# yihua7/NeRF-Texture

Measured on AMD Instinct MI355X. Metric: ray-samples/s (train), higher is better.
Workload: dtype f16

## Files before the change

nerf-texture_amd/csrc/common.hpp:

```cpp
#pragma once

#include <hip/hip_runtime.h>
#include <hip/hip_fp16.h>
#include <stdint.h>

#include <cstdarg>
#include <cstdio>

#include "../../include/nerftex_hip.h"

namespace nerftex {

void set_error(const char* fmt, ...);
void clear_error();

inline hipStream_t as_stream(void* s) { return reinterpret_cast<hipStream_t>(s); }

inline int check_launch(const char* what) {
    hipError_t e = hipGetLastError();
    if (e != hipSuccess) {
        set_error("%s: HIP launch failed: %s", what, hipGetErrorString(e));
        return NERFTEX_ERR_HIP;
    }
    return NERFTEX_OK;
}

#define NERFTEX_HIP_TRY(expr, what)                                                   \
    do {                                                                              \
        hipError_t _e = (expr);                                                       \
        if (_e != hipSuccess) {                                                       \
            ::nerftex::set_error("%s: %s", what, hipGetErrorString(_e));              \
            return NERFTEX_ERR_HIP;                                                   \
        }                                                                             \
    } while (0)

template <typename T>
constexpr T div_up(T a, T b) { return (a + b - 1) / b; }

inline int device_cus() {
    static int cus[16] = {0};
    int dev = 0;
    if (hipGetDevice(&dev) != hipSuccess || dev < 0 || dev >= 16) return 256;
    if (cus[dev] == 0) {
        hipDeviceProp_t prop;
        cus[dev] = (hipGetDeviceProperties(&prop, dev) == hipSuccess && prop.multiProcessorCount > 0) ? prop.multiProcessorCount : 256;
    }
    return cus[dev];
}

enum Knob {
    kKnobGridFwd,
    kKnobGridBwd,
    kKnobGridBwdSweep,
    kKnobGridBwdItems,
    kKnobGridBwdSlice,
    kKnobGridBwdNoMerge,
    kKnobGridBwdProbe,
    kKnobMarch,
    kKnobMarchSerial,
    kKnobFfmlpWgPerCu,
    kKnobFfmlpBwdSplit,
    kKnobMarchLean,
    kKnobFfmlpBwdTr,
    kKnobGridBwdStage,
    kKnobCompositeKeep,
    kKnobMarchCountProbe,
    kKnobPlanarLanes,
    kKnobPatchLanes,
    kKnobCount
};
extern long g_knobs[kKnobCount];
inline long knob(Knob k) { return g_knobs[k]; }

extern int g_profile_mode;
constexpr int kTimeAny = 1, kTimeGrid = 2;
void profile_begin(const char* name, hipStream_t st, int* slot);
void profile_end(hipStream_t st, int slot);
struct KernelTimer {
    hipStream_t st;
    int slot = -1;
    KernelTimer(const char* name, hipStream_t s, int group = kTimeAny) : st(s) {
        if (g_profile_mode == 1 || (g_profile_mode == 2 && group == kTimeGrid)) profile_begin(name, s, &slot);
    }
    ~KernelTimer() { if (slot >= 0) profile_end(st, slot); }
};

using half_t = _Float16;
typedef _Float16 half2_t __attribute__((ext_vector_type(2)));
typedef _Float16 half4_t __attribute__((ext_vector_type(4)));
typedef _Float16 half8_t __attribute__((ext_vector_type(8)));
typedef float float2_t __attribute__((ext_vector_type(2)));
typedef float float4_t __attribute__((ext_vector_type(4)));
typedef float float16_t __attribute__((ext_vector_type(16)));

constexpr int kWave = 64;

__host__ __device__ __forceinline__ uint32_t unit_rows(uint32_t code, uint32_t count) {
    if (!(code >> 31)) return code;
    const uint32_t F = (code >> 24) & 127u, N = code & 0xffffffu;
    const uint32_t q = F * N / (count ? count : 1u);
    return q < F ? F : (q > 8u * F ? 8u * F : q);
}
__device__ __forceinline__ uint32_t live_rows(uint32_t B, const int32_t* __restrict__ units_dev, uint32_t rows_per_unit) {
    if (!units_dev) return B;
    const uint32_t n = (uint32_t)units_dev[0];
    return min(B, n * unit_rows(rows_per_unit, n));
}
__device__ __forceinline__ bool slot_unused(const float* __restrict__ dirs, size_t row) { return dirs[row * 3] > 1e29f; }

}
```

nerf-texture_amd/csrc/ffmlp_body.inc:

```

constexpr int kBlockThreads = 256;
constexpr int kTilesPerWave = 2;
constexpr int kRowsPerBlock = 4 * 16 * kTilesPerWave;
constexpr float kAct = 10.0f;

enum Act : uint32_t { kRelu = 0, kExp = 1, kSine = 2, kSigmoid = 3, kSquareplus = 4, kSoftplus = 5, kNone = 6 };

__device__ __forceinline__ float act_forward(uint32_t a, float x) {
    switch (a) {
        case kRelu: return __builtin_bit_cast(float, max(__builtin_bit_cast(int, x), 0));
        case kExp: return expf(x);
        case kSine: return sinf(x);
        case kSigmoid: return 1.0f / (1.0f + expf(-x));
        case kSquareplus: { const float s = x * kAct; return 0.5f * (s + sqrtf(s * s + 4.0f)) / kAct; }
        case kSoftplus: return logf(expf(x * kAct) + 1.0f) / kAct;
        default: return x;
    }
}
__device__ __forceinline__ float act_backward(uint32_t a, float g, float y) {
    switch (a) {
        case kRelu: return y > 0.0f ? g : 0.0f;
        case kExp: return g * y;
        case kSigmoid: return g * (float)(elem_t)(y * (1.0f - y));
        case kSquareplus: { const float s = y * kAct; return g * (float)(elem_t)(s * s / (s * s + 1.0f)); }
        case kSoftplus: return g * (float)(elem_t)(1.0f - expf(-y * kAct));
        default: return g;
    }
}

template <int ACT>
__device__ __forceinline__ float act_fwd(uint32_t act_rt, float x) {
    if constexpr (ACT >= 0) return act_forward((uint32_t)ACT, x);
    else return act_forward(act_rt, x);
}
template <int ACT>
__device__ __forceinline__ float act_bwd(uint32_t act_rt, float g, float y) {
    if constexpr (ACT >= 0) return act_backward((uint32_t)ACT, g, y);
    else return act_backward(act_rt, g, y);
}


__device__ __forceinline__ int kmap(bool permuted, int ks, int g, int j) {
    return permuted ? 32 * ks + 16 * (j >> 2) + 4 * g + (j & 3) : 32 * ks + 8 * g + j;
}

__device__ void stage_fragments(elem8_t* __restrict__ dst, const elem_t* __restrict__ W, int ldw, bool transposed, int M, int K,
                                bool permuted) {
    const int KS = (K + 31) / 32;
    const elem8_t zero8{0, 0, 0, 0, 0, 0, 0, 0};
    if (!transposed) {
        const int total = (M / 16) * KS * 64;
        for (int s = threadIdx.x; s < total; s += kBlockThreads) {
            const int frag = s >> 6, lane = s & 63;
            const int mt = frag / KS, ks = frag - mt * KS;
            const int m = 16 * mt + (lane & 15), g = lane >> 4;
            const elem_t* row = W + (size_t)m * ldw;
            elem8_t v;
            if (!permuted) {
                const int k0 = 32 * ks + 8 * g;
                v = k0 < K ? *reinterpret_cast<const elem8_t*>(row + k0) : zero8;
            } else {
                const int ka = 32 * ks + 4 * g, kb = ka + 16;
                const elem4_t z4{0, 0, 0, 0};
                const elem4_t lo = ka < K ? *reinterpret_cast<const elem4_t*>(row + ka) : z4;
                const elem4_t hi = kb < K ? *reinterpret_cast<const elem4_t*>(row + kb) : z4;
                v = elem8_t{lo[0], lo[1], lo[2], lo[3], hi[0], hi[1], hi[2], hi[3]};
            }
            dst[s] = v;
        }
    } else {
        elem_t* d = reinterpret_cast<elem_t*>(dst);
        const int MP = M / 8;
        for (int s = threadIdx.x; s < KS * 32 * MP; s += kBlockThreads) {
            const int k = s / MP, m0 = 8 * (s - k * MP);
            const elem8_t v = k < K ? *reinterpret_cast<const elem8_t*>(W + (size_t)k * ldw + m0) : zero8;
            const int ks = k >> 5, kk = k & 31;
            const int g = permuted ? (kk & 15) >> 2 : kk >> 3;
            const int j = permuted ? 4 * (kk >> 4) + (kk & 3) : kk & 7;
#pragma unroll
            for (int i = 0; i < 8; i++) {
                const int m = m0 + i;
                d[((size_t)((m >> 4) * KS + ks) * 64 + (m & 15) + 16 * g) * 8 + j] = v[i];
            }
        }
    }
}

__host__ __device__ constexpr int frag_count(int M, int K) { return (M / 16) * ((K + 31) / 32); }

__device__ __forceinline__ elem8_t pack_operand(const float4_t& lo, const float4_t& hi) {
    elem8_t b;
#pragma unroll
    for (int j = 0; j < 4; j++) {
        b[j] = (elem_t)lo[j];
        b[4 + j] = (elem_t)hi[j];
    }
    return b;
}

__device__ __forceinline__ void store4(elem_t* p, const float4_t& v) {
    elem4_t h;
#pragma unroll
    for (int j = 0; j < 4; j++) h[j] = (elem_t)v[j];
    *reinterpret_cast<elem4_t*>(p) = h;
}

template <int HIDDEN, bool INFERENCE, bool STAGED, int ACT, int OUT_ACT, bool STREAM = false, bool ROWS = false>
__global__ __launch_bounds__(kBlockThreads) void ffmlp_forward_kernel(const elem_t* __restrict__ X, const elem_t* __restrict__ W,
                                                                      elem_t* __restrict__ fwd, elem_t* __restrict__ out, uint32_t B,
                                                                      uint32_t IN, uint32_t NL, uint32_t act, uint32_t out_act,
                                                                      const int32_t* __restrict__ units_dev, uint32_t rows_per_unit) {
    constexpr int OT = HIDDEN / 16;
    constexpr int KSH = (HIDDEN + 31) / 32;
    constexpr int NT = kTilesPerWave;
    uint32_t live = B;
    if constexpr (ROWS) {
        live = live_rows(B, units_dev, rows_per_unit);
        if (blockIdx.x * kRowsPerBlock >= live) return;
    }
    extern __shared__ __attribute__((aligned(16))) char smem[];
    elem8_t* frags = reinterpret_cast<elem8_t*>(smem);

    const int KS0 = (IN + 31) / 32;
    const int base_hidden = OT * KS0;
    const int per_hidden = OT * KSH;
    const int base_out = base_hidden + (NL - 1) * per_hidden;
    const size_t patch_offset = (size_t)(base_out + KSH) * 1024;
    static_assert(!(STREAM && STAGED), "the streaming form stores its activations directly (the LDS holds one layer's fragments and nothing else)");
    if constexpr (!STREAM) {
        stage_fragments(frags, W, IN, false, HIDDEN, IN, false);
        for (uint32_t l = 1; l < NL; l++)
            stage_fragments(frags + (size_t)(base_hidden + (l - 1) * per_hidden) * 64, W + (size_t)HIDDEN * IN + (size_t)(l - 1) * HIDDEN * HIDDEN,
                            HIDDEN, false, HIDDEN, HIDDEN, true);
        stage_fragments(frags + (size_t)base_out * 64, W + (size_t)HIDDEN * IN + (size_t)(NL - 1) * HIDDEN * HIDDEN, HIDDEN, false, 16, HIDDEN,
                        true);
        __syncthreads();
    }
    auto fragments_of = [&](uint32_t m) -> const elem8_t* {
        if constexpr (STREAM) {
            __syncthreads();
            if (m == 0) stage_fragments(frags, W, IN, false, HIDDEN, IN, false);
            else if (m < NL) stage_fragments(frags, W + (size_t)HIDDEN * IN + (size_t)(m - 1) * HIDDEN * HIDDEN, HIDDEN, false, HIDDEN, HIDDEN, true);
            else stage_fragments(frags, W + (size_t)HIDDEN * IN + (size_t)(NL - 1) * HIDDEN * HIDDEN, HIDDEN, false, 16, HIDDEN, true);
            __syncthreads();
            return frags;
        } else {
            return m == 0 ? frags : (m < NL ? frags + (size_t)(base_hidden + (m - 1) * per_hidden) * 64 : frags + (size_t)base_out * 64);
        }
    };

    const int wave = threadIdx.x >> 6, lane = threadIdx.x & 63, r = lane & 15, g = lane >> 4;
    const size_t layer_stride = (size_t)B * HIDDEN;
    constexpr int kRowPitch = HIDDEN + 8;
    elem_t* patch = reinterpret_cast<elem_t*>(smem + patch_offset) + (size_t)wave * 16 * NT * kRowPitch;

    for (uint32_t row0 = blockIdx.x * kRowsPerBlock + wave * 16 * NT; ROWS ? row0 - wave * 16 * NT < live : row0 < B; row0 += gridDim.x * kRowsPerBlock) {
        float4_t acc[NT][OT];
#pragma unroll
        for (int t = 0; t < NT; t++)
#pragma unroll
            for (int ot = 0; ot < OT; ot++) acc[t][ot] = float4_t{0, 0, 0, 0};

        const elem8_t* f0 = fragments_of(0);
        for (int ks = 0; ks < KS0; ks++) {
            elem8_t b[NT];
            const uint32_t k0 = 32 * ks + 8 * g;
#pragma unroll
            for (int t = 0; t < NT; t++) {
                if (k0 < IN) b[t] = *reinterpret_cast<const elem8_t*>(X + (size_t)(row0 + 16 * t + r) * IN + k0);
                else b[t] = elem8_t{0, 0, 0, 0, 0, 0, 0, 0};
            }
#pragma unroll
            for (int ot = 0; ot < OT; ot++) {
                const elem8_t a = f0[(size_t)(ot * KS0 + ks) * 64 + lane];
#pragma unroll
                for (int t = 0; t < NT; t++) acc[t][ot] = mfma16(a, b[t], acc[t][ot]);
            }
        }

        elem8_t bop[NT][KSH];
        for (uint32_t l = 0;; l++) {
#pragma unroll
            for (int t = 0; t < NT; t++) {
#pragma unroll
                for (int ot = 0; ot < OT; ot++) {
#pragma unroll
                    for (int j = 0; j < 4; j++) acc[t][ot][j] = act_fwd<ACT>(act, acc[t][ot][j]);
                    if constexpr (!INFERENCE) {
                        if constexpr (STAGED) store4(patch + (size_t)(16 * t + r) * kRowPitch + 16 * ot + 4 * g, acc[t][ot]);
                        else store4(fwd + l * layer_stride + (size_t)(row0 + 16 * t + r) * HIDDEN + 16 * ot + 4 * g, acc[t][ot]);
                    }
                }
#pragma unroll
                for (int s = 0; s < KSH; s++) {
                    const float4_t zero{0, 0, 0, 0};
                    bop[t][s] = pack_operand(acc[t][2 * s], (2 * s + 1 < OT) ? acc[t][(2 * s + 1 < OT) ? 2 * s + 1 : 0] : zero);
                }
            }
            if constexpr (!INFERENCE && STAGED) {
                constexpr int kPieces = HIDDEN / 8;
                elem_t* dst = fwd + l * layer_stride + (size_t)row0 * HIDDEN;
#pragma unroll
                for (int it = 0; it < 16 * NT * kPieces / 64; it++) {
                    const int c = it * 64 + lane, row = c / kPieces, piece = c % kPieces;
                    *reinterpret_cast<elem8_t*>(dst + (size_t)row * HIDDEN + 8 * piece) =
                        *reinterpret_cast<const elem8_t*>(patch + (size_t)row * kRowPitch + 8 * piece);
                }
            }
            if (l + 1 >= NL) break;
            const elem8_t* fl = fragments_of(l + 1);
#pragma unroll
            for (int ot = 0; ot < OT; ot++) {
                float4_t c[NT];
#pragma unroll
                for (int t = 0; t < NT; t++) c[t] = float4_t{0, 0, 0, 0};
#pragma unroll
                for (int ks = 0; ks < KSH; ks++) {
                    const elem8_t a = fl[(size_t)(ot * KSH + ks) * 64 + lane];
#pragma unroll
                    for (int t = 0; t < NT; t++) c[t] = mfma16(a, bop[t][ks], c[t]);
                }
#pragma unroll
                for (int t = 0; t < NT; t++) acc[t][ot] = c[t];
            }
        }

        {
            const elem8_t* fo = fragments_of(NL);
            float4_t c[NT];
#pragma unroll
            for (int t = 0; t < NT; t++) c[t] = float4_t{0, 0, 0, 0};
#pragma unroll
            for (int ks = 0; ks < KSH; ks++) {
                const elem8_t a = fo[(size_t)ks * 64 + lane];
#pragma unroll
                for (int t = 0; t < NT; t++) c[t] = mfma16(a, bop[t][ks], c[t]);
            }
#pragma unroll
            for (int t = 0; t < NT; t++) {
#pragma unroll
                for (int j = 0; j < 4; j++) c[t][j] = act_fwd<OUT_ACT>(out_act, c[t][j]);
                store4(out + (size_t)(row0 + 16 * t + r) * 16 + 4 * g, c[t]);
            }
        }
    }
}

__device__ __forceinline__ elem_t narrow16(float v) {
    asm volatile("" : "+v"(v));
    return (elem_t)v;
}

template <bool TRAIN, bool DENSITY = false>
__global__ __launch_bounds__(kBlockThreads) void field_forward_kernel(const elem_t* __restrict__ feats, const float* __restrict__ dirs,
                                                                      const elem_t* __restrict__ Ws, const elem_t* __restrict__ Wc, uint32_t B,
                                                                      float* __restrict__ sigma, float* __restrict__ rgbs, elem_t* __restrict__ x_rows,
                                                                      elem_t* __restrict__ h_out, elem_t* __restrict__ cin_out,
                                                                      elem_t* __restrict__ hc_out, const int* __restrict__ units_dev,
                                                                      uint32_t rows_per_unit) {
    constexpr int HIDDEN = 64, IN = 32, OT = 4, KSH = 2, NT = kTilesPerWave;
    const uint32_t live = units_dev ? min(B, (uint32_t)units_dev[0] * unit_rows(rows_per_unit, (uint32_t)units_dev[0])) : B;
    extern __shared__ __attribute__((aligned(16))) char smem[];
    elem8_t* frags = reinterpret_cast<elem8_t*>(smem);
    constexpr int kS0 = 0, kS1 = 4, kSo = 12, kC0 = 14, kC1 = 18, kC2 = 26, kCo = 34;
    stage_fragments(frags + kS0 * 64, Ws, IN, false, HIDDEN, IN, false);
    stage_fragments(frags + kS1 * 64, Ws + HIDDEN * IN, HIDDEN, false, HIDDEN, HIDDEN, true);
    stage_fragments(frags + kSo * 64, Ws + HIDDEN * IN + HIDDEN * HIDDEN, HIDDEN, false, 16, HIDDEN, true);
    if constexpr (!DENSITY) {
        stage_fragments(frags + kC0 * 64, Wc, IN, false, HIDDEN, IN, false);
        stage_fragments(frags + kC1 * 64, Wc + HIDDEN * IN, HIDDEN, false, HIDDEN, HIDDEN, true);
        stage_fragments(frags + kC2 * 64, Wc + HIDDEN * IN + HIDDEN * HIDDEN, HIDDEN, false, HIDDEN, HIDDEN, true);
        stage_fragments(frags + kCo * 64, Wc + HIDDEN * IN + 2 * HIDDEN * HIDDEN, HIDDEN, false, 16, HIDDEN, true);
    }
    __syncthreads();

    const int wave = threadIdx.x >> 6, lane = threadIdx.x & 63, r = lane & 15, g = lane >> 4;
    auto hidden = [&](const elem8_t* fl, const elem8_t (&bop)[NT][KSH], float4_t (&acc)[NT][OT]) {
#pragma unroll
        for (int ot = 0; ot < OT; ot++) {
            float4_t c[NT];
#pragma unroll
            for (int t = 0; t < NT; t++) c[t] = float4_t{0, 0, 0, 0};
#pragma unroll
            for (int ks = 0; ks < KSH; ks++) {
                const elem8_t a = fl[(size_t)(ot * KSH + ks) * 64 + lane];
#pragma unroll
                for (int t = 0; t < NT; t++) c[t] = mfma16(a, bop[t][ks], c[t]);
            }
#pragma unroll
            for (int t = 0; t < NT; t++) acc[t][ot] = c[t];
        }
    };
    auto relu_pack = [&](float4_t (&acc)[NT][OT], elem8_t (&bop)[NT][KSH]) {
#pragma unroll
        for (int t = 0; t < NT; t++) {
#pragma unroll
            for (int ot = 0; ot < OT; ot++)
#pragma unroll
                for (int j = 0; j < 4; j++) acc[t][ot][j] = act_forward(kRelu, acc[t][ot][j]);
#pragma unroll
            for (int s = 0; s < KSH; s++) bop[t][s] = pack_operand(acc[t][2 * s], acc[t][2 * s + 1]);
        }
    };
    auto out_tile = [&](const elem8_t* fo, const elem8_t (&bop)[NT][KSH], float4_t (&c)[NT]) {
#pragma unroll
        for (int t = 0; t < NT; t++) c[t] = float4_t{0, 0, 0, 0};
#pragma unroll
        for (int ks = 0; ks < KSH; ks++) {
            const elem8_t a = fo[(size_t)ks * 64 + lane];
#pragma unroll
            for (int t = 0; t < NT; t++) c[t] = mfma16(a, bop[t][ks], c[t]);
        }
    };

    for (uint32_t row0 = blockIdx.x * kRowsPerBlock + wave * 16 * NT; row0 < live; row0 += gridDim.x * kRowsPerBlock) {
        if constexpr (!TRAIN && !DENSITY) {
            bool used = false;
#pragma unroll
            for (int t = 0; t < NT; t++) used |= !(dirs[(size_t)(row0 + 16 * t + r) * 3] > 1e29f);
            if (__ballot(used) == 0ull) continue;
        }
        float4_t acc[NT][OT];
        elem8_t bop[NT][KSH];
        {
            elem8_t b[NT];
#pragma unroll
            for (int t = 0; t < NT; t++) {
                const size_t row = row0 + 16 * t + r;
                uint32_t w[4];
#pragma unroll
                for (int q = 0; q < 4; q++) w[q] = *reinterpret_cast<const uint32_t*>(feats + ((size_t)(4 * g + q) * B + row) * 2);
                typedef uint32_t u4 __attribute__((ext_vector_type(4)));
                if constexpr (kElemIsHalf) {
                    b[t] = __builtin_bit_cast(elem8_t, u4{w[0], w[1], w[2], w[3]});
                } else {
                    const half8_t hf = __builtin_bit_cast(half8_t, u4{w[0], w[1], w[2], w[3]});
#pragma unroll
                    for (int j = 0; j < 8; j++) b[t][j] = (elem_t)(float)hf[j];
                }
                if constexpr (TRAIN) *reinterpret_cast<elem8_t*>(x_rows + row * IN + 8 * g) = b[t];
            }
#pragma unroll
            for (int ot = 0; ot < OT; ot++) {
                const elem8_t a = frags[(size_t)(kS0 + ot) * 64 + lane];
#pragma unroll
                for (int t = 0; t < NT; t++) acc[t][ot] = mfma16(a, b[t], float4_t{0, 0, 0, 0});
            }
        }
        relu_pack(acc, bop);
        hidden(frags + kS1 * 64, bop, acc);
        relu_pack(acc, bop);
        float4_t h[NT];
        out_tile(frags + kSo * 64, bop, h);

        if constexpr (DENSITY) {
            if (g == 0) {
#pragma unroll
                for (int t = 0; t < NT; t++) sigma[row0 + 16 * t + r] = expf((float)(elem_t)h[t][0]);
            }
            continue;
        }
        elem8_t bc[NT];
#pragma unroll
        for (int t = 0; t < NT; t++) {
            const size_t row = row0 + 16 * t + r;
            float4_t hr;
#pragma unroll
            for (int j = 0; j < 4; j++) hr[j] = (float)(elem_t)h[t][j];
            if (g == 0) sigma[row] = expf(hr[0]);
            float sh16[16];
            sh::eval<4>(dirs[row * 3], dirs[row * 3 + 1], dirs[row * 3 + 2], sh16);
            elem8_t cv;
#pragma unroll
            for (int j = 0; j < 8; j++) {
                const float geo = __shfl(hr[(j + 1) & 3], r + 16 * (2 * (g & 1) + ((j + 1) >> 2)), 64);
                float sh_lo = sh16[j], sh_hi = sh16[8 + j];
                asm volatile("" : "+v"(sh_lo), "+v"(sh_hi));
                const float shj = (g & 1) ? sh_hi : sh_lo;
                cv[j] = g < 2 ? narrow16(shj) : ((g == 3 && j == 7) ? (elem_t)0.0f : (elem_t)geo);
            }
            bc[t] = cv;
            if constexpr (TRAIN) {
                store4(h_out + row * 16 + 4 * g, h[t]);
                *reinterpret_cast<elem8_t*>(cin_out + row * IN + 8 * g) = cv;
            }
        }
#pragma unroll
        for (int ot = 0; ot < OT; ot++) {
            const elem8_t a = frags[(size_t)(kC0 + ot) * 64 + lane];
#pragma unroll
            for (int t = 0; t < NT; t++) acc[t][ot] = mfma16(a, bc[t], float4_t{0, 0, 0, 0});
        }
        relu_pack(acc, bop);
        hidden(frags + kC1 * 64, bop, acc);
        relu_pack(acc, bop);
        hidden(frags + kC2 * 64, bop, acc);
        relu_pack(acc, bop);
        float4_t c[NT];
        out_tile(frags + kCo * 64, bop, c);
#pragma unroll
        for (int t = 0; t < NT; t++) {
            const size_t row = row0 + 16 * t + r;
            if constexpr (TRAIN)
                if (hc_out) store4(hc_out + row * 16 + 4 * g, c[t]);
            if (g == 0) {
#pragma unroll
                for (int k = 0; k < 3; k++) {
                    const float x = (float)(elem_t)c[t][k];
                    rgbs[row * 3 + k] = (float)narrow16(1.0f / (1.0f + expf(-x)));
                }
            }
        }
    }
}

template <int HIDDEN, bool STREAM = false>
__global__ __launch_bounds__(kBlockThreads) void ffmlp_dgrad_kernel(const elem_t* __restrict__ grad, const elem_t* __restrict__ W,
                                                                    const elem_t* __restrict__ fwd, elem_t* __restrict__ bb,
                                                                    elem_t* __restrict__ grad_inputs, uint32_t B, uint32_t IN, uint32_t NL,
                                                                    uint32_t act) {
    constexpr int OT = HIDDEN / 16;
    constexpr int KSH = (HIDDEN + 31) / 32;
    constexpr int NT = kTilesPerWave;
    extern __shared__ __attribute__((aligned(16))) char smem[];
    elem8_t* frags = reinterpret_cast<elem8_t*>(smem);

    const elem_t* W_hidden = W + (size_t)HIDDEN * IN;
    const elem_t* W_out = W_hidden + (size_t)(NL - 1) * HIDDEN * HIDDEN;
    const int per_hidden = OT * KSH;
    const int base_hidden = OT;
    const int base_in = base_hidden + (NL - 1) * per_hidden;
    if constexpr (!STREAM) {
        stage_fragments(frags, W_out, HIDDEN, true, HIDDEN, 16, false);
        for (uint32_t j = 1; j < NL; j++)
            stage_fragments(frags + (size_t)(base_hidden + (j - 1) * per_hidden) * 64, W_hidden + (size_t)(NL - 1 - j) * HIDDEN * HIDDEN, HIDDEN, true,
                            HIDDEN, HIDDEN, true);
        if (grad_inputs) stage_fragments(frags + (size_t)base_in * 64, W, IN, true, IN, HIDDEN, true);
        __syncthreads();
    }
    auto fragments_of = [&](uint32_t j) -> const elem8_t* {
        if constexpr (STREAM) {
            __syncthreads();
            if (j == 0) stage_fragments(frags, W_out, HIDDEN, true, HIDDEN, 16, false);
            else if (j < NL) stage_fragments(frags, W_hidden + (size_t)(NL - 1 - j) * HIDDEN * HIDDEN, HIDDEN, true, HIDDEN, HIDDEN, true);
            else stage_fragments(frags, W, IN, true, IN, HIDDEN, true);
            __syncthreads();
            return frags;
        } else {
            return j == 0 ? frags : (j < NL ? frags + (size_t)(base_hidden + (j - 1) * per_hidden) * 64 : frags + (size_t)base_in * 64);
        }
    };

    const int wave = threadIdx.x >> 6, lane = threadIdx.x & 63, r = lane & 15, g = lane >> 4;
    const size_t layer_stride = (size_t)B * HIDDEN;

    for (uint32_t row0 = blockIdx.x * kRowsPerBlock + wave * 16 * NT; row0 < B; row0 += gridDim.x * kRowsPerBlock) {
        elem8_t bg[NT];
#pragma unroll
        for (int t = 0; t < NT; t++) {
            if (g < 2) bg[t] = *reinterpret_cast<const elem8_t*>(grad + (size_t)(row0 + 16 * t + r) * 16 + 8 * g);
            else bg[t] = elem8_t{0, 0, 0, 0, 0, 0, 0, 0};
        }
        float4_t acc[NT][OT];
        const elem8_t* fout = fragments_of(0);
#pragma unroll
        for (int ot = 0; ot < OT; ot++) {
            const elem8_t a = fout[(size_t)ot * 64 + lane];
#pragma unroll
            for (int t = 0; t < NT; t++) acc[t][ot] = mfma16(a, bg[t], float4_t{0, 0, 0, 0});
        }

        elem8_t bop[NT][KSH];
        for (uint32_t j = 0;; j++) {
            const elem_t* f = fwd + (size_t)(NL - 1 - j) * layer_stride;
#pragma unroll
            for (int t = 0; t < NT; t++) {
#pragma unroll
                for (int ot = 0; ot < OT; ot++) {
                    const size_t off = (size_t)(row0 + 16 * t + r) * HIDDEN + 16 * ot + 4 * g;
                    const elem4_t y = *reinterpret_cast<const elem4_t*>(f + off);
#pragma unroll
                    for (int q = 0; q < 4; q++) acc[t][ot][q] = act_backward(act, (float)(elem_t)acc[t][ot][q], (float)y[q]);
                    store4(bb + j * layer_stride + off, acc[t][ot]);
                }
#pragma unroll
                for (int s = 0; s < KSH; s++) {
                    const float4_t zero{0, 0, 0, 0};
                    bop[t][s] = pack_operand(acc[t][2 * s], (2 * s + 1 < OT) ? acc[t][(2 * s + 1 < OT) ? 2 * s + 1 : 0] : zero);
                }
            }
            if (j + 1 >= NL) break;
            const elem8_t* fl = fragments_of(j + 1);
#pragma unroll
            for (int ot = 0; ot < OT; ot++) {
                float4_t c[NT];
// ... 918 lines not shown
        return NERFTEX_ERR_INVALID;
    }
    return dispatch_forward<false>(inputs, weights, B, input_dim, hidden_dim, num_layers, activation, output_activation, forward_buffer, outputs,
                                   as_stream(stream));
}

int inference_entry(const void* inputs, const void* weights, uint32_t B, uint32_t input_dim, uint32_t output_dim,
                                       uint32_t hidden_dim, uint32_t num_layers, uint32_t activation, uint32_t output_activation,
                                       void* inference_buffer, void* outputs, void* stream) {
    (void)inference_buffer;
    clear_error();
    int rc = validate(B, input_dim, output_dim, hidden_dim, num_layers, activation, output_activation);
    if (rc != NERFTEX_OK || B == 0) return rc;
    if ((rc = weights_aligned(weights)) != NERFTEX_OK) return rc;
    return dispatch_forward<true>(inputs, weights, B, input_dim, hidden_dim, num_layers, activation, output_activation, nullptr, outputs,
                                  as_stream(stream));
}

int backward_entry(const void* grad, const void* inputs, const void* weights, const void* forward_buffer, uint32_t B,
                                      uint32_t input_dim, uint32_t output_dim, uint32_t hidden_dim, uint32_t num_layers, uint32_t activation,
                                      uint32_t output_activation, int calc_grad_inputs, void* backward_buffer, void* grad_inputs,
                                      void* grad_weights, void* stream) {
    clear_error();
    int rc = validate(B, input_dim, output_dim, hidden_dim, num_layers, activation, output_activation);
    if (rc != NERFTEX_OK || B == 0) return rc;
    if ((rc = weights_aligned(weights)) != NERFTEX_OK) return rc;

    hipStream_t st = as_stream(stream);
    const uint32_t H = hidden_dim, IN = input_dim, NL = num_layers;
    void* gi = calc_grad_inputs ? grad_inputs : nullptr;
    const uint32_t n_params = H * (IN + H * (NL - 1) + 16);

    {
        if (!knob(kKnobFfmlpBwdSplit)) {
            rc = launch_backward_fused(grad, inputs, weights, forward_buffer, gi, B, IN, H, NL, activation, n_params, grad_weights, st);
            if (rc >= 0) return rc;
        }
    }
    if (!backward_buffer || !forward_buffer) {
        set_error("ffmlp_backward: forward_buffer and backward_buffer must not be NULL for this shape / mode");
        return NERFTEX_ERR_INVALID;
    }

    switch (H) {
        case 16: rc = launch_dgrad<16>(grad, weights, forward_buffer, backward_buffer, gi, B, IN, NL, activation, st); break;
        case 32: rc = launch_dgrad<32>(grad, weights, forward_buffer, backward_buffer, gi, B, IN, NL, activation, st); break;
        case 64: rc = launch_dgrad<64>(grad, weights, forward_buffer, backward_buffer, gi, B, IN, NL, activation, st); break;
        case 128: rc = launch_dgrad<128>(grad, weights, forward_buffer, backward_buffer, gi, B, IN, NL, activation, st); break;
        default: rc = launch_dgrad<256>(grad, weights, forward_buffer, backward_buffer, gi, B, IN, NL, activation, st); break;
    }
    if (rc != NERFTEX_OK) return rc;

    const size_t LS = (size_t)B * H;
    const elem_t* fb = static_cast<const elem_t*>(forward_buffer);
    const elem_t* bb = static_cast<const elem_t*>(backward_buffer);
    WgradArgs args{};
    args.layer[0] = WgradLayer{bb + (size_t)(NL - 1) * LS, static_cast<const elem_t*>(inputs), H, IN, H, IN, 0};
    for (uint32_t l = 1; l < NL; l++)
        args.layer[l] = WgradLayer{bb + (size_t)(NL - 1 - l) * LS, fb + (size_t)(l - 1) * LS, H, H, H, H, H * IN + (l - 1) * H * H};
    args.layer[NL] = WgradLayer{static_cast<const elem_t*>(grad), fb + (size_t)(NL - 1) * LS, 16, H, 16, H, H * IN + (NL - 1) * H * H};

    uint32_t n_parts = B / 128;
    const uint32_t cap = (uint32_t)num_cus() / 2;
    if (n_parts > cap) n_parts = cap;
    if (n_parts == 0) n_parts = 1;
    float* partials = static_cast<float*>(workspace(kWsMlp, sizeof(float) * (size_t)n_parts * n_params, st));
    if (!partials) return NERFTEX_ERR_HIP;
    const size_t red_bytes = sizeof(float) * 4 * 16 * 256;
    {
        KernelTimer kt("ffmlp_wgrad_kernel", st);
        hipLaunchKernelGGL(ffmlp_wgrad_kernel, dim3(n_parts, NL + 1), dim3(kBlockThreads), red_bytes, st, args, B, partials, n_params);
    }
    rc = check_launch("ffmlp_backward(wgrad)");
    if (rc != NERFTEX_OK) return rc;
    {
        KernelTimer kt("ffmlp_wgrad_reduce_kernel", st);
        hipLaunchKernelGGL(ffmlp_wgrad_reduce_kernel, dim3(div_up(n_params, kRedParams)), dim3(kBlockThreads), 0, st, partials, n_parts,
                           n_params, static_cast<elem_t*>(grad_weights));
    }
    return check_launch("ffmlp_backward(reduce)");
}


int field_density_entry(const void* feats_lbc, const void* sigma_weights, uint32_t B, float* sigma, void* stream) {
    clear_error();
    if (B % kRowsPerBlock != 0) {
        set_error("field_density: the batch must be a multiple of %d rows", kRowsPerBlock);
        return NERFTEX_ERR_INVALID;
    }
    if (B == 0) return NERFTEX_OK;
    int rc = weights_aligned(sigma_weights);
    if (rc != NERFTEX_OK) return rc;
    const size_t lds = (size_t)14 * 1024;
    hipStream_t st = as_stream(stream);
    {
        KernelTimer kt("field_density_kernel", st);
        hipLaunchKernelGGL((field_forward_kernel<false, true>), dim3(persistent_grid(B, lds)), dim3(kBlockThreads), lds, st, (const elem_t*)feats_lbc,
                           (const float*)nullptr, (const elem_t*)sigma_weights, (const elem_t*)nullptr, B, sigma, (float*)nullptr, (elem_t*)nullptr,
                           (elem_t*)nullptr, (elem_t*)nullptr, (elem_t*)nullptr, (const int*)nullptr, 0u);
    }
    return check_launch("field_density");
}

int field_forward_entry(const void* feats_lbc, const float* dirs, const void* sigma_weights, const void* color_weights, uint32_t B, float* sigma,
                        float* rgbs, void* x_rows, void* h, void* cin, void* hc, const int32_t* units_dev, uint32_t rows_per_unit, void* stream) {
    clear_error();
    if (B % kRowsPerBlock != 0) {
        set_error("field_forward: the batch must be a multiple of %d rows", kRowsPerBlock);
        return NERFTEX_ERR_INVALID;
    }
    const bool train = x_rows || h || cin || hc;
    if (train && !(x_rows && h && cin)) {
        set_error("field_forward: x_rows, h and cin (and optionally hc) are written together (training) or not at all (inference)");
        return NERFTEX_ERR_INVALID;
    }
    if (B == 0) return NERFTEX_OK;
    int rc = weights_aligned(sigma_weights);
    if (rc == NERFTEX_OK) rc = weights_aligned(color_weights);
    if (rc != NERFTEX_OK) return rc;
    const size_t lds = (size_t)36 * 1024;
    auto kernel = train ? field_forward_kernel<true> : field_forward_kernel<false>;
    hipStream_t st = as_stream(stream);
    {
        KernelTimer kt(train ? "field_forward_train_kernel" : "field_forward_kernel", st);
        hipLaunchKernelGGL(kernel, dim3(persistent_grid(B, lds)), dim3(kBlockThreads), lds, st, (const elem_t*)feats_lbc, dirs, (const elem_t*)sigma_weights,
                           (const elem_t*)color_weights, B, sigma, rgbs, (elem_t*)x_rows, (elem_t*)h, (elem_t*)cin, (elem_t*)hc, units_dev, rows_per_unit);
    }
    return check_launch("field_forward");
}
```

nerf-texture_amd/csrc/runtime.hip:

```cpp
#include "common.hpp"
#include "workspace.hpp"

#include <atomic>

#include <cstdlib>
#include <cstring>
#include <map>
#include <mutex>
#include <string>
#include <vector>

namespace nerftex {

static thread_local char g_err[512] = {0};

void set_error(const char* fmt, ...) {
    va_list ap;
    va_start(ap, fmt);
    vsnprintf(g_err, sizeof(g_err), fmt, ap);
    va_end(ap);
}

void clear_error() { g_err[0] = 0; }

long g_knobs[kKnobCount] = {0};
namespace {
const char* const kKnobNames[kKnobCount] = {"grid_fwd", "grid_bwd", "grid_bwd_sweep", "grid_bwd_items", "grid_bwd_slice", "grid_bwd_nomerge",
                                            "grid_bwd_probe", "march", "march_serial", "ffmlp_wg_per_cu",
                                            "ffmlp_bwd_split", "march_lean", "ffmlp_bwd_tr", "grid_bwd_stage", "composite_keep", "march_count_probe", "planar_lanes",
                                            "patch_lanes"};
int knob_index(const char* name, size_t n) {
    for (int k = 0; k < kKnobCount; k++)
        if (strlen(kKnobNames[k]) == n && strncmp(kKnobNames[k], name, n) == 0) return k;
    return -1;
}
struct KnobInit {
    KnobInit() {
        auto env = [](const char* n) { const char* v = getenv(n); return v ? v : ""; };
        const char* v;
        v = env("NERFTEX_GRID_FWD"); g_knobs[kKnobGridFwd] = v[0] == 'p' ? 1 : v[0] == 'l' ? 2 : 0;
        v = env("NERFTEX_GRID_BWD"); g_knobs[kKnobGridBwd] = v[0] == 'a' ? 1 : v[0] == 'o' ? 2 : 0;
        g_knobs[kKnobGridBwdSweep] = env("NERFTEX_GRID_BWD_ALGO")[0] == 's';
        g_knobs[kKnobGridBwdItems] = atol(env("NERFTEX_GRID_BWD_ITEMS"));
        g_knobs[kKnobGridBwdSlice] = atol(env("NERFTEX_GRID_BWD_SLICE"));
        g_knobs[kKnobGridBwdNoMerge] = getenv("NERFTEX_GRID_BWD_NOMERGE") != nullptr;
        v = env("NERFTEX_MARCH"); g_knobs[kKnobMarch] = v[0] == 'r' ? 1 : v[0] == 'l' ? 2 : 0;
        g_knobs[kKnobMarchSerial] = env("NERFTEX_MARCH_COUNT")[0] == 's';
        g_knobs[kKnobFfmlpWgPerCu] = atol(env("NERFTEX_FFMLP_WG_PER_CU"));
        g_knobs[kKnobFfmlpBwdSplit] = env("NERFTEX_FFMLP_BWD")[0] == 's';
        for (const char* p = env("NERFTEX_TUNE"); *p;) {
            const char* eq = strchr(p, '=');
            if (!eq) break;
            const int k = knob_index(p, (size_t)(eq - p));
            if (k >= 0) g_knobs[k] = atol(eq + 1);
            const char* c = strchr(eq, ',');
            if (!c) break;
            p = c + 1;
        }
    }
} g_knob_init;
}

namespace {
constexpr int kMaxDevices = 16;
struct Slot { void* ptr = nullptr; size_t bytes = 0; };
struct SlotSet { Slot slot[kWsSlots]; };
std::map<hipStream_t, SlotSet> g_ws[kMaxDevices];
const hipStream_t kCaptureSet = reinterpret_cast<hipStream_t>(~(uintptr_t)0);
std::vector<void*> g_retired;
std::mutex g_ws_mutex;
}

std::atomic<unsigned> g_ws_touched{0};
thread_local int t_capture_set = 0;

void* workspace(WorkspaceSlot slot, size_t bytes, hipStream_t stream) {
    g_ws_touched.fetch_or(1u << (unsigned)slot, std::memory_order_relaxed);
    int dev = 0;
    if (hipGetDevice(&dev) != hipSuccess || dev < 0 || dev >= kMaxDevices) {
        set_error("workspace: bad device");
        return nullptr;
    }
    hipStreamCaptureStatus cap = hipStreamCaptureStatusNone;
    if (hipStreamIsCapturing(stream, &cap) == hipSuccess && cap != hipStreamCaptureStatusNone)
        stream = reinterpret_cast<hipStream_t>(reinterpret_cast<uintptr_t>(kCaptureSet) - (uintptr_t)t_capture_set);
    std::lock_guard<std::mutex> lock(g_ws_mutex);
    Slot& s = g_ws[dev][stream].slot[slot];
    if (s.bytes < bytes) {
        if (s.ptr) g_retired.push_back(s.ptr);
        s.ptr = nullptr;
        s.bytes = 0;
        size_t want = bytes < (1u << 20) ? (1u << 20) : bytes + bytes / 2;
        hipStreamCaptureMode mode = hipStreamCaptureModeRelaxed;
        (void)hipThreadExchangeStreamCaptureMode(&mode);
        const hipError_t err = hipMalloc(&s.ptr, want);
        (void)hipThreadExchangeStreamCaptureMode(&mode);
        if (err != hipSuccess) {
            set_error("workspace: hipMalloc(%zu) failed", want);
            s.ptr = nullptr;
            return nullptr;
        }
        s.bytes = want;
        static const int poison = [] { const char* v = getenv("NERFTEX_POISON_WORKSPACE"); return v && *v ? atoi(v) : -1; }();
        if (poison >= 0) {
            (void)hipThreadExchangeStreamCaptureMode(&mode);
            (void)hipMemset(s.ptr, poison & 255, want);
            (void)hipThreadExchangeStreamCaptureMode(&mode);
        }
    }
    return s.ptr;
}

bool peek_workspace(int slot, hipStream_t stream, void** ptr, size_t* bytes) {
// ... 147 lines not shown
```

Measured before the change: 938.6 million.

## Prefetch next rows and stage weight fragments directly in field forward kernel

Restructures the fused field MLP forward kernel so each wave loads its weight fragments straight from global memory into LDS slots instead of the generic staging loop. Features and directions for the next grid-stride step are prefetched while the current step computes. Blocks with no live rows exit early. Spherical-harmonic packing is done once per step via permlane32 swaps, and the geometry features are shuffled as packed halves, cutting per-tile shuffles and conversions. It also adds compile-time probe variants, selected by a knob that defaults to off. The risks are higher register pressure from the prefetch buffers and a changed LDS layout.

```diff
diff --git a/nerf-texture_amd/csrc/common.hpp b/nerf-texture_amd/csrc/common.hpp
--- a/nerf-texture_amd/csrc/common.hpp
+++ b/nerf-texture_amd/csrc/common.hpp
@@ -67,6 +67,7 @@
     kKnobMarchCountProbe,
     kKnobPlanarLanes,
     kKnobPatchLanes,
+    kKnobFieldFwdProbe,
     kKnobCount
 };
 extern long g_knobs[kKnobCount];
diff --git a/nerf-texture_amd/csrc/ffmlp_body.inc b/nerf-texture_amd/csrc/ffmlp_body.inc
--- a/nerf-texture_amd/csrc/ffmlp_body.inc
+++ b/nerf-texture_amd/csrc/ffmlp_body.inc
@@ -88,6 +88,19 @@
 
 __host__ __device__ constexpr int frag_count(int M, int K) { return (M / 16) * ((K + 31) / 32); }
 
+template <int KS, bool PERMUTED>
+__device__ __forceinline__ elem8_t fragment_slot(const elem_t* __restrict__ W, int ldw, int f, int lane) {
+    const int mt = f / KS, ks = f - mt * KS;
+    const elem_t* row = W + (size_t)(16 * mt + (lane & 15)) * ldw + 32 * ks;
+    const int g = lane >> 4;
+    if constexpr (!PERMUTED) {
+        return *reinterpret_cast<const elem8_t*>(row + 8 * g);
+    } else {
+        const elem4_t lo = *reinterpret_cast<const elem4_t*>(row + 4 * g), hi = *reinterpret_cast<const elem4_t*>(row + 4 * g + 16);
+        return elem8_t{lo[0], lo[1], lo[2], lo[3], hi[0], hi[1], hi[2], hi[3]};
+    }
+}
+
 __device__ __forceinline__ elem8_t pack_operand(const float4_t& lo, const float4_t& hi) {
     elem8_t b;
 #pragma unroll
@@ -251,7 +264,12 @@
     return (elem_t)v;
 }
 
-template <bool TRAIN, bool DENSITY = false>
+enum FieldProbe : int { kProbeOff = 0, kProbeStaging = 1, kProbeLoads = 2, kProbeSigma = 3, kProbeMid = 4, kProbeColour = 5, kProbeCount = 6 };
+typedef uint32_t uint4_t __attribute__((ext_vector_type(4)));
+__device__ __forceinline__ void probe_sink(const elem8_t& v) { asm volatile("" ::"v"(__builtin_bit_cast(uint4_t, v))); }
+__device__ __forceinline__ void probe_sink(const float4_t& v) { asm volatile("" ::"v"(v)); }
+
+template <bool TRAIN, bool DENSITY = false, int PROBE = kProbeOff>
 __global__ __launch_bounds__(kBlockThreads) void field_forward_kernel(const elem_t* __restrict__ feats, const float* __restrict__ dirs,
                                                                       const elem_t* __restrict__ Ws, const elem_t* __restrict__ Wc, uint32_t B,
                                                                       float* __restrict__ sigma, float* __restrict__ rgbs, elem_t* __restrict__ x_rows,
@@ -259,22 +277,76 @@
                                                                       elem_t* __restrict__ hc_out, const int* __restrict__ units_dev,
                                                                       uint32_t rows_per_unit) {
     constexpr int HIDDEN = 64, IN = 32, OT = 4, KSH = 2, NT = kTilesPerWave;
+    constexpr bool SKIP = !TRAIN && !DENSITY;
     const uint32_t live = units_dev ? min(B, (uint32_t)units_dev[0] * unit_rows(rows_per_unit, (uint32_t)units_dev[0])) : B;
+    if (blockIdx.x * kRowsPerBlock >= live) return;
     extern __shared__ __attribute__((aligned(16))) char smem[];
     elem8_t* frags = reinterpret_cast<elem8_t*>(smem);
-    constexpr int kS0 = 0, kS1 = 4, kSo = 12, kC0 = 14, kC1 = 18, kC2 = 26, kCo = 34;
-    stage_fragments(frags + kS0 * 64, Ws, IN, false, HIDDEN, IN, false);
-    stage_fragments(frags + kS1 * 64, Ws + HIDDEN * IN, HIDDEN, false, HIDDEN, HIDDEN, true);
-    stage_fragments(frags + kSo * 64, Ws + HIDDEN * IN + HIDDEN * HIDDEN, HIDDEN, false, 16, HIDDEN, true);
-    if constexpr (!DENSITY) {
-        stage_fragments(frags + kC0 * 64, Wc, IN, false, HIDDEN, IN, false);
-        stage_fragments(frags + kC1 * 64, Wc + HIDDEN * IN, HIDDEN, false, HIDDEN, HIDDEN, true);
-        stage_fragments(frags + kC2 * 64, Wc + HIDDEN * IN + HIDDEN * HIDDEN, HIDDEN, false, HIDDEN, HIDDEN, true);
-        stage_fragments(frags + kCo * 64, Wc + HIDDEN * IN + 2 * HIDDEN * HIDDEN, HIDDEN, false, 16, HIDDEN, true);
+
+    const int wave = __builtin_amdgcn_readfirstlane(threadIdx.x >> 6), lane = threadIdx.x & 63, r = lane & 15, g = lane >> 4;
+    const uint32_t stride = gridDim.x * kRowsPerBlock;
+    struct Feat { uint32_t w[NT][4]; };
+    struct Dir { float x, y, z; };
+    auto load_feats = [&](uint32_t row0) {
+        Feat f;
+#pragma unroll
+        for (int t = 0; t < NT; t++)
+#pragma unroll
+            for (int q = 0; q < 4; q++) f.w[t][q] = *reinterpret_cast<const uint32_t*>(feats + ((size_t)(4 * g + q) * B + row0 + 16 * t + r) * 2);
+        return f;
+    };
+    auto load_dir = [&](uint32_t row0) {
+        Dir d{0.0f, 0.0f, 0.0f};
+        if constexpr (!DENSITY) {
+            const size_t row = row0 + 16 * (g >> 1) + r;
+            d = Dir{dirs[row * 3], dirs[row * 3 + 1], dirs[row * 3 + 2]};
+        }
+        return d;
+    };
+    auto step_used = [&](const Dir& d) {
+        if constexpr (SKIP) return __ballot(!(d.x > 1e29f)) != 0ull;
+        else return true;
+    };
+    uint32_t row0 = blockIdx.x * kRowsPerBlock + wave * 16 * NT, row1 = row0 + stride;
+    const bool any_step = row0 < live;
+    if (!any_step) row0 = row1 = blockIdx.x * kRowsPerBlock;
+    Dir d_cur = load_dir(row0), d_nxt = load_dir(row1 < live ? row1 : row0);
+    bool used_cur = step_used(d_cur);
+    Feat w_cur = load_feats(row0);
+
+    constexpr int kS0 = 0, kS1 = 4, kC0 = 12, kC1 = 16, kC2 = 24, kSo = DENSITY ? 12 : 32, kCo = 34;
+    {
+        constexpr int kGroups = DENSITY ? 4 : 9;
+        const elem_t* const Ws1 = Ws + HIDDEN * IN;
+        const elem_t* const Wso = Ws1 + HIDDEN * HIDDEN;
+        elem8_t fv[kGroups];
+        fv[0] = fragment_slot<1, false>(Ws, IN, wave, lane);
+        fv[1] = fragment_slot<2, true>(Ws1, HIDDEN, wave, lane);
+        fv[2] = fragment_slot<2, true>(Ws1, HIDDEN, 4 + wave, lane);
+        if constexpr (DENSITY) {
+            fv[3] = fragment_slot<2, true>(Wso, HIDDEN, wave & 1, lane);
+        } else {
+            const elem_t* const Wc1 = Wc + HIDDEN * IN;
+            const elem_t* const Wc2 = Wc1 + HIDDEN * HIDDEN;
+            fv[3] = fragment_slot<1, false>(Wc, IN, wave, lane);
+            fv[4] = fragment_slot<2, true>(Wc1, HIDDEN, wave, lane);
+            fv[5] = fragment_slot<2, true>(Wc1, HIDDEN, 4 + wave, lane);
+            fv[6] = fragment_slot<2, true>(Wc2, HIDDEN, wave, lane);
+            fv[7] = fragment_slot<2, true>(Wc2, HIDDEN, 4 + wave, lane);
+            fv[8] = fragment_slot<2, true>(wave < 2 ? Wso : Wc2 + HIDDEN * HIDDEN, HIDDEN, wave & 1, lane);
+        }
+#pragma unroll
+        for (int t = 0; t < NT; t++)
+#pragma unroll
+            for (int q = 0; q < 4; q++) asm volatile("" : "+v"(w_cur.w[t][q]));
+        asm volatile("" : "+v"(d_cur.x), "+v"(d_cur.y), "+v"(d_cur.z), "+v"(d_nxt.x), "+v"(d_nxt.y), "+v"(d_nxt.z));
+#pragma unroll
+        for (int i = 0; i < kGroups; i++)
+            if (!DENSITY || i < 3 || wave < 2) frags[(size_t)(4 * i + wave) * 64 + lane] = fv[i];
     }
     __syncthreads();
-
-    const int wave = threadIdx.x >> 6, lane = threadIdx.x & 63, r = lane & 15, g = lane >> 4;
+    if (PROBE == kProbeStaging || !any_step) return;
+
     auto hidden = [&](const elem8_t* fl, const elem8_t (&bop)[NT][KSH], float4_t (&acc)[NT][OT]) {
 #pragma unroll
         for (int ot = 0; ot < OT; ot++) {
@@ -313,13 +385,7 @@
         }
     };
 
-    for (uint32_t row0 = blockIdx.x * kRowsPerBlock + wave * 16 * NT; row0 < live; row0 += gridDim.x * kRowsPerBlock) {
-        if constexpr (!TRAIN && !DENSITY) {
-            bool used = false;
-#pragma unroll
-            for (int t = 0; t < NT; t++) used |= !(dirs[(size_t)(row0 + 16 * t + r) * 3] > 1e29f);
-            if (__ballot(used) == 0ull) continue;
-        }
+    auto step = [&](const uint32_t row0, const Feat& in, const Dir& dir) {
         float4_t acc[NT][OT];
         elem8_t bop[NT][KSH];
         {
@@ -327,18 +393,20 @@
 #pragma unroll
             for (int t = 0; t < NT; t++) {
                 const size_t row = row0 + 16 * t + r;
-                uint32_t w[4];
-#pragma unroll
-                for (int q = 0; q < 4; q++) w[q] = *reinterpret_cast<const uint32_t*>(feats + ((size_t)(4 * g + q) * B + row) * 2);
-                typedef uint32_t u4 __attribute__((ext_vector_type(4)));
+                const uint4_t w{in.w[t][0], in.w[t][1], in.w[t][2], in.w[t][3]};
                 if constexpr (kElemIsHalf) {
-                    b[t] = __builtin_bit_cast(elem8_t, u4{w[0], w[1], w[2], w[3]});
+                    b[t] = __builtin_bit_cast(elem8_t, w);
                 } else {
-                    const half8_t hf = __builtin_bit_cast(half8_t, u4{w[0], w[1], w[2], w[3]});
+                    const half8_t hf = __builtin_bit_cast(half8_t, w);
 #pragma unroll
                     for (int j = 0; j < 8; j++) b[t][j] = (elem_t)(float)hf[j];
                 }
                 if constexpr (TRAIN) *reinterpret_cast<elem8_t*>(x_rows + row * IN + 8 * g) = b[t];
+            }
+            if constexpr (PROBE == kProbeLoads) {
+#pragma unroll
+                for (int t = 0; t < NT; t++) probe_sink(b[t]);
+                return;
             }
 #pragma unroll
             for (int ot = 0; ot < OT; ot++) {
@@ -352,38 +420,69 @@
         relu_pack(acc, bop);
         float4_t h[NT];
         out_tile(frags + kSo * 64, bop, h);
+        if constexpr (PROBE == kProbeSigma) {
+#pragma unroll
+            for (int t = 0; t < NT; t++) probe_sink(h[t]);
+            return;
+        }
 
         if constexpr (DENSITY) {
             if (g == 0) {
 #pragma unroll
                 for (int t = 0; t < NT; t++) sigma[row0 + 16 * t + r] = expf((float)(elem_t)h[t][0]);
             }
-            continue;
+            return;
+        }
+        uint4_t sh_part[NT];
+        {
+            float sh16[16];
+            sh::eval<4>(dir.x, dir.y, dir.z, sh16);
+            elem8_t sv;
+#pragma unroll
+            for (int j = 0; j < 8; j++) {
+                float sh_lo = sh16[j], sh_hi = sh16[8 + j];
+                asm volatile("" : "+v"(sh_lo), "+v"(sh_hi));
+                sv[j] = narrow16((g & 1) ? sh_hi : sh_lo);
+            }
+            const uint4_t own = __builtin_bit_cast(uint4_t, sv);
+#pragma unroll
+            for (int q = 0; q < 4; q++) {
+                const auto halves = __builtin_amdgcn_permlane32_swap(own[q], own[q], false, false);
+                sh_part[0][q] = halves[0];
+                sh_part[1][q] = halves[1];
+            }
         }
         elem8_t bc[NT];
 #pragma unroll
         for (int t = 0; t < NT; t++) {
             const size_t row = row0 + 16 * t + r;
-            float4_t hr;
-#pragma unroll
-            for (int j = 0; j < 4; j++) hr[j] = (float)(elem_t)h[t][j];
-            if (g == 0) sigma[row] = expf(hr[0]);
-            float sh16[16];
-            sh::eval<4>(dirs[row * 3], dirs[row * 3 + 1], dirs[row * 3 + 2], sh16);
-            elem8_t cv;
-#pragma unroll
-            for (int j = 0; j < 8; j++) {
-                const float geo = __shfl(hr[(j + 1) & 3], r + 16 * (2 * (g & 1) + ((j + 1) >> 2)), 64);
-                float sh_lo = sh16[j], sh_hi = sh16[8 + j];
-                asm volatile("" : "+v"(sh_lo), "+v"(sh_hi));
-                const float shj = (g & 1) ? sh_hi : sh_lo;
-                cv[j] = g < 2 ? narrow16(shj) : ((g == 3 && j == 7) ? (elem_t)0.0f : (elem_t)geo);
-            }
-            bc[t] = cv;
+            elem4_t hh;
+#pragma unroll
+            for (int j = 0; j < 4; j++) hh[j] = (elem_t)h[t][j];
+            if (g == 0) sigma[row] = expf((float)hh[0]);
+            typedef uint32_t uint2_t __attribute__((ext_vector_type(2)));
+            const uint2_t hp = __builtin_bit_cast(uint2_t, hh);
+            const int src = r + 32 * (g & 1);
+            uint32_t s[5];
+            s[0] = __shfl(hp[0], src, 64);
+            s[1] = __shfl(hp[1], src, 64);
+            s[2] = __shfl(hp[0], src + 16, 64);
+            s[3] = __shfl(hp[1], src + 16, 64);
+            s[4] = __shfl(hp[0], (src + 32) & 63, 64);
+            if (g & 1) s[4] = 0u;
+            uint4_t cv;
+#pragma unroll
+            for (int q = 0; q < 4; q++) cv[q] = g < 2 ? sh_part[t][q] : __builtin_amdgcn_alignbit(s[q + 1], s[q], 16);
+            bc[t] = __builtin_bit_cast(elem8_t, cv);
             if constexpr (TRAIN) {
-                store4(h_out + row * 16 + 4 * g, h[t]);
-                *reinterpret_cast<elem8_t*>(cin_out + row * IN + 8 * g) = cv;
-            }
+                *reinterpret_cast<elem4_t*>(h_out + row * 16 + 4 * g) = hh;
+                *reinterpret_cast<elem8_t*>(cin_out + row * IN + 8 * g) = bc[t];
+            }
+        }
+        if constexpr (PROBE == kProbeMid) {
+#pragma unroll
+            for (int t = 0; t < NT; t++) probe_sink(bc[t]);
+            return;
         }
 #pragma unroll
         for (int ot = 0; ot < OT; ot++) {
@@ -398,6 +497,11 @@
         relu_pack(acc, bop);
         float4_t c[NT];
         out_tile(frags + kCo * 64, bop, c);
+        if constexpr (PROBE == kProbeColour) {
+#pragma unroll
+            for (int t = 0; t < NT; t++) probe_sink(c[t]);
+            return;
+        }
 #pragma unroll
         for (int t = 0; t < NT; t++) {
             const size_t row = row0 + 16 * t + r;
@@ -411,6 +515,17 @@
                 }
             }
         }
+    };
+
+    while (true) {
+        const uint32_t row2 = row1 + stride;
+        const bool used_nxt = row1 < live && step_used(d_nxt);
+        const Feat w_nxt = load_feats(used_nxt ? row1 : row0);
+        const Dir d_nn = load_dir(row2 < live ? row2 : row0);
+        if (used_cur) step(row0, w_cur, d_cur);
+        if (row1 >= live) break;
+        row0 = row1, row1 = row2;
+        w_cur = w_nxt, d_cur = d_nxt, d_nxt = d_nn, used_cur = used_nxt;
     }
 }
 
@@ -1495,6 +1610,14 @@
 }
 
 
+using FieldForwardFn = void (*)(const elem_t*, const float*, const elem_t*, const elem_t*, uint32_t, float*, float*, elem_t*, elem_t*, elem_t*, elem_t*,
+                                const int*, uint32_t);
+template <bool TRAIN, bool DENSITY, int PROBE = kProbeCount - 1>
+FieldForwardFn field_forward_variant(long probe) {
+    if constexpr (PROBE == kProbeOff) return field_forward_kernel<TRAIN, DENSITY, kProbeOff>;
+    else return probe == PROBE ? field_forward_kernel<TRAIN, DENSITY, PROBE> : field_forward_variant<TRAIN, DENSITY, PROBE - 1>(probe);
+}
+
 int field_density_entry(const void* feats_lbc, const void* sigma_weights, uint32_t B, float* sigma, void* stream) {
     clear_error();
     if (B % kRowsPerBlock != 0) {
@@ -1508,7 +1631,8 @@
     hipStream_t st = as_stream(stream);
     {
         KernelTimer kt("field_density_kernel", st);
-        hipLaunchKernelGGL((field_forward_kernel<false, true>), dim3(persistent_grid(B, lds)), dim3(kBlockThreads), lds, st, (const elem_t*)feats_lbc,
+        const FieldForwardFn kernel = field_forward_variant<false, true>(knob(kKnobFieldFwdProbe));
+        hipLaunchKernelGGL(kernel, dim3(persistent_grid(B, lds)), dim3(kBlockThreads), lds, st, (const elem_t*)feats_lbc,
                            (const float*)nullptr, (const elem_t*)sigma_weights, (const elem_t*)nullptr, B, sigma, (float*)nullptr, (elem_t*)nullptr,
                            (elem_t*)nullptr, (elem_t*)nullptr, (elem_t*)nullptr, (const int*)nullptr, 0u);
     }
@@ -1532,7 +1656,7 @@
     if (rc == NERFTEX_OK) rc = weights_aligned(color_weights);
     if (rc != NERFTEX_OK) return rc;
     const size_t lds = (size_t)36 * 1024;
-    auto kernel = train ? field_forward_kernel<true> : field_forward_kernel<false>;
+    auto kernel = train ? field_forward_variant<true, false>(knob(kKnobFieldFwdProbe)) : field_forward_variant<false, false>(knob(kKnobFieldFwdProbe));
     hipStream_t st = as_stream(stream);
     {
         KernelTimer kt(train ? "field_forward_train_kernel" : "field_forward_kernel", st);
diff --git a/nerf-texture_amd/csrc/runtime.hip b/nerf-texture_amd/csrc/runtime.hip
--- a/nerf-texture_amd/csrc/runtime.hip
+++ b/nerf-texture_amd/csrc/runtime.hip
@@ -28,7 +28,7 @@
 const char* const kKnobNames[kKnobCount] = {"grid_fwd", "grid_bwd", "grid_bwd_sweep", "grid_bwd_items", "grid_bwd_slice", "grid_bwd_nomerge",
                                             "grid_bwd_probe", "march", "march_serial", "ffmlp_wg_per_cu",
                                             "ffmlp_bwd_split", "march_lean", "ffmlp_bwd_tr", "grid_bwd_stage", "composite_keep", "march_count_probe", "planar_lanes",
-                                            "patch_lanes"};
+                                            "patch_lanes", "field_fwd_probe"};
 int knob_index(const char* name, size_t n) {
     for (int k = 0; k < kKnobCount; k++)
         if (strlen(kKnobNames[k]) == n && strncmp(kKnobNames[k], name, n) == 0) return k;
```

Result: no change. 946.8 million, median of 6 (+0.9%).
